# vpc-ccg/circminer

Hardware: AMD Instinct MI355X
Metric: paired reads/sec (whole node), hg38 k=20, 2x150 bp; circ_report bit-exact (higher is better)
Workload: dtype int32/u8 (chain scores f64)

## Files before the change

circminer_amd/csrc/cm_core.h:

```cpp
#pragma once
#include <stdint.h>

#include "circminer_hot.h"
#if defined(CM_STAGE2_HOST)
#include <vector>
#endif

#if defined(__HIPCC__)
#define CM_HD __host__ __device__
#define CM_NOINLINE inline
#else
#define CM_HD
#define CM_NOINLINE
#endif

#if !defined(CM_HOOK_DP)
#define CM_HOOK_DP(kind, s, n, t, m) ((void)0)
#endif
#if defined(CM_STATS) && !defined(__HIPCC__)
#if !defined(CM_NSTATS)
#define CM_NSTATS 16
#endif
extern "C" unsigned long long cm_stats[CM_NSTATS];
#define CM_STAT(i, n) ((i) < CM_NSTATS ? (void)(cm_stats[(i) < CM_NSTATS ? (i) : 0] += (unsigned long long)(n)) : (void)0)
// ... 59 lines not shown
};
struct AnnotV {
    uint32_t n_iv, n_seg, n_trans, n_gene, n_chr, iv_bucket_shift, n_iv_bucket, pair_reach;
    uint64_t n_bits;
    const CM_G IvRec *iv;
    g_u32 iv_seg;
    const CM_G SegRec *seg;
    g_u32 seg_tid;
    const CM_G TrRec *tr;
    g_u8 t2s;
    const CM_G GeneRec *gene;
    g_u64 near_border_bits, intronic_bits;
    g_u32 chr_shift;
    g_i32 chr_id;
    g_u32 iv_bucket;
};
CM_HD inline IndexV to_dev(const cm_index_view &v) {
    IndexV d;
    d.contig_num = v.contig_num; d.ref_len = v.ref_len; d.n_entries = v.n_entries;
    d.genome = (g_u8)v.genome; d.bucket_off = (g_u32)v.bucket_off; d.checksum = (g_u16)v.checksum; d.pos = (g_u32)v.pos;
    return d;
}
CM_HD inline AnnotV to_dev(const AnnotDev &v) {
    AnnotV d;
    d.n_iv = v.n_iv; d.n_seg = v.n_seg; d.n_trans = v.n_trans; d.n_gene = v.n_gene; d.n_chr = v.n_chr;
    d.iv_bucket_shift = v.iv_bucket_shift; d.n_iv_bucket = v.n_iv_bucket; d.n_bits = v.n_bits; d.pair_reach = v.pair_reach;
    d.iv = (const CM_G IvRec *)v.iv; d.iv_seg = (g_u32)v.iv_seg; d.seg = (const CM_G SegRec *)v.seg; d.seg_tid = (g_u32)v.seg_tid;
    d.tr = (const CM_G TrRec *)v.tr; d.t2s = (g_u8)v.t2s; d.gene = (const CM_G GeneRec *)v.gene;
    d.near_border_bits = (g_u64)v.near_border_bits; d.intronic_bits = (g_u64)v.intronic_bits;
    d.chr_shift = (g_u32)v.chr_shift; d.chr_id = (g_i32)v.chr_id; d.iv_bucket = (g_u32)v.iv_bucket;
    return d;
}

constexpr int INF_I = 1000000000;
constexpr uint32_t MINLB = 0u;
constexpr uint32_t MAXUB = 4294967295u;
constexpr int MAXDISCRDTLEN = 20000;
constexpr uint32_t LARIAT2BEGTH = 1000u;
constexpr int DPTINF = 10000000;
constexpr int SC_MAT = 1, SC_MIS = -3, SC_IND = -3, SC_XD = 8;
constexpr int MAX_SEEDS = CM_MAX_CHAIN_FRAGS;
constexpr int MAX_BAND = 8;
constexpr int MAX_TID = 64;
#if defined(CM_STAGE2_HOST)
constexpr int MEMO_N = 512;
#elif defined(CM_MEMO_N)
constexpr int MEMO_N = CM_MEMO_N;
#else
constexpr int MEMO_N = 8;
#endif

enum { ERR_POOL = 1, ERR_SEEDS = 4, ERR_BAND = 8, ERR_MEMO = 16 };

struct KCore {
    cm_params P;
    cm_index_view X;
    AnnotDev A;
    const uint32_t *desc = nullptr;
    const uint64_t *entry_near = nullptr;
};
struct Core {
    cm_params P;
    IndexV X;
    AnnotV A;
    g_u32 desc = nullptr;
    g_u64 entry_near = nullptr;
};
CM_HD inline Core to_core(const KCore &k) {
    Core c;
    c.P = k.P;
    c.X = to_dev(k.X);
    c.A = to_dev(k.A);
    c.desc = (g_u32)k.desc;
    c.entry_near = (g_u64)k.entry_near;
    return c;
}

template <class T> CM_HD inline T cmin(T a, T b) { return a < b ? a : b; }
template <class T> CM_HD inline T cmax(T a, T b) { return a > b ? a : b; }
CM_HD inline int cabs(int a) { return a < 0 ? -a : a; }

struct SV {
    g_u8 p;
    int32_t off;
    int32_t step;
    int32_t mode;
    CM_HD inline SV sub(int a) const { return SV{p, off + a * step, step, mode}; }
    CM_HD inline SV rev(int m) const { return SV{p, off + (m - 1) * step, -step, mode}; }
};
struct Read {
    g_u8 p;
    int32_t len;
    int32_t rc;
    CM_HD inline SV view() const { return rc ? SV{p, len - 1, -1, 1} : SV{p, 0, 1, 0}; }
};


struct Probe {
    uint32_t start;
    uint32_t raw;
    uint32_t touches;
};
template <class AT> CM_HD inline void probe_search(const AT &at, uint32_t n, int target, uint32_t b0, Probe &r) {
    uint32_t lb = 1, ub = n, mid;
    while (lb < ub) {
        mid = (lb + ub) / 2;
        ++r.touches;
        if (target <= at(mid - 1)) ub = mid;
        else lb = mid + 1;
    }
    ++r.touches;
    if (ub < lb || target != at(lb - 1)) return;
    const uint32_t LB = lb;
    uint32_t UB = lb;
    ub = n;
    while (lb < ub) {
        mid = (lb + ub + 1) / 2;
        ++r.touches;
        if (target < at(mid - 1)) ub = mid - 1;
        else lb = mid;
    }
    ++r.touches;
    if (target == at(lb - 1)) UB = lb;
    r.start = b0 + (LB - 1);
    r.raw = UB - LB + 1;
}
constexpr int DESC_WORDS = 4;
CM_HD inline int desc_cbits(int kmer) { return 2 * (kmer - CM_WINDOW_SIZE); }
CM_HD inline uint32_t desc_inline(int kmer) { return desc_cbits(kmer) > 0 ? (uint32_t)(88 / desc_cbits(kmer)) : 254u; }
CM_HD inline int desc_value(uint32_t d1, uint32_t d2, uint32_t d3, uint32_t i, int cbits) {
    const uint32_t sh = 8u + i * (uint32_t)cbits, w = sh >> 5, bit = sh & 31u;
    const uint32_t lo = w == 0 ? d1 : (w == 1 ? d2 : d3), hi = w == 0 ? d2 : (w == 1 ? d3 : 0u);
    const uint64_t two = ((uint64_t)hi << 32) | lo;
    return (int)((uint32_t)(two >> bit) & ((1u << cbits) - 1u));
}
template <class CK> CM_HD inline void desc_pack(uint32_t b0, uint32_t n, const CK &cks , int kmer, uint32_t out[DESC_WORDS]) {
    const int cbits = desc_cbits(kmer);
    uint64_t lo = n < 255u ? n : 255u;
    uint32_t hi = 0;
    if (n <= desc_inline(kmer) && cbits > 0)
        for (uint32_t i = 0; i < n; ++i) {
            const uint32_t sh = 8u + i * (uint32_t)cbits;
            const uint64_t v = (uint64_t)(cks(i) & ((1u << cbits) - 1u));
            if (sh < 64u) {
                lo |= v << sh;
                if (sh + (uint32_t)cbits > 64u) hi |= (uint32_t)(v >> (64u - sh));
            } else hi |= (uint32_t)(v << (sh - 64u));
        }
    out[0] = b0;
    out[1] = (uint32_t)lo;
    out[2] = (uint32_t)(lo >> 32);
    out[3] = hi;
}
CM_HD inline Probe seed_probe(const Core &c, const SV &s, int qpos) {
    Probe r{0u, 0u, 0u};
    int hv = 0, cv = 0;
    uint32_t bad = 0;
    const uint32_t rc = s.mode == 1 ? 1u : 0u;
    for (int i = 0; i < c.P.kmer; ++i) {
        uint32_t u = s.mode == 2 ? 0u : (uint32_t)s.p[s.off + (qpos + i) * s.step];
        u = rc ? (u & 0xDFu) : u;
        bad |= (uint32_t)!((u == 'A') | (u == 'C') | (u == 'G') | (u == 'T'));
        uint32_t code = ((u >> 1) ^ (u >> 2)) & 3u;
        code = rc ? 3u - code : code;
        if (i < CM_WINDOW_SIZE) hv = (hv << 2) | (int)code;
        else cv = (cv << 2) | (int)code;
    }
    if (bad) return r;
    const int target = (int)(int16_t)cv;
    if (c.desc) {
        const g_u32 d = c.desc + (uint64_t)(uint32_t)hv * DESC_WORDS;
        uint32_t w[DESC_WORDS];
        __builtin_memcpy(w, (const CM_G uint8_t *)d, sizeof(w));
        const uint32_t n8 = w[1] & 0xffu;
        if (n8 == 0) return r;
        if (n8 <= desc_inline(c.P.kmer)) {
            const int cbits = desc_cbits(c.P.kmer);
            const uint32_t d1 = w[1], d2 = w[2], d3 = w[3];
            probe_search([&](uint32_t i) { return cbits > 0 ? desc_value(d1, d2, d3, i, cbits) : 0; }, n8, target, w[0], r);
            return r;
        }
    }
    const uint32_t b0 = c.X.bucket_off[hv], b1 = c.X.bucket_off[hv + 1];
    if (b1 == b0) return r;
    const g_u16 it = c.X.checksum + b0;
    probe_search([&](uint32_t i) { return (int)it[i]; }, b1 - b0, target, b0, r);
    return r;
}

CM_HD inline bool bit_at(g_u64 b, uint64_t n, uint64_t p) { return p < n && ((b[p >> 6] >> (p & 63)) & 1ull); }
CM_HD inline uint32_t iv_nseg(const AnnotV &A, int iv) { return A.iv[iv].nseg; }
CM_HD inline uint32_t iv_segid(const AnnotV &A, int iv, uint32_t i) { return A.iv_seg[A.iv[iv].seg_off + i]; }

CM_HD inline int iv_find_ind(const AnnotV &A, uint32_t pos, int &ind) {
    CM_STAT(10, 1);
    ind = -1;
    if (pos < A.iv[0].spos) return -1;
    int beg = 0, end = (int)A.n_iv;
    const uint32_t b = pos >> A.iv_bucket_shift;
    if (A.iv_bucket && b + 1 < A.n_iv_bucket) {
        beg = (int)A.iv_bucket[b];
        end = (int)A.iv_bucket[b + 1];
        if (beg > 0) --beg;
        if (end < (int)A.n_iv) ++end;
        if (end <= beg) end = beg + 1;
    }
    while (end - beg > 1) {
        const int mid = (beg + end) / 2;
        if (pos < A.iv[mid].spos) end = mid;
        else beg = mid;
    }
    ind = end - 1;
    if (ind < 0 || A.iv[ind].epos < pos) return -1;
    return ind;
}
CM_HD inline int overlap_ind(const Core &c, uint32_t loc, int &ind) {
    int r = iv_find_ind(c.A, loc, ind);
    if (r < 0 || iv_nseg(c.A, r) == 0) return -1;
    return r;
}
CM_HD inline int overlap(const Core &c, uint32_t loc) { int ind; return overlap_ind(c, loc, ind); }

CM_HD inline uint32_t upper_bound_lookup(const Core &c, uint32_t spos, uint32_t mlen, uint32_t rlen, uint32_t &max_end, int &ol) {
    const AnnotV &A = c.A;
    max_end = 0;
    int it_ind = -1;
    int ov = iv_find_ind(A, spos, it_ind);
    const uint32_t epos = spos + mlen - 1;
    if (ov < 0 || iv_nseg(A, ov) == 0) {
        ol = -1;
        int nx = it_ind + 1;
        max_end = ((nx < 0 || nx >= (int)A.n_iv) ? 0u : A.iv[nx].spos) - 1u;
        if (max_end < epos) return 0;
        return cmin(spos + rlen + (uint32_t)c.P.max_ed, max_end - mlen + 1);
    }
    ol = -1;
    uint32_t min_end = 1000000000u, max_next = 0;
    if (epos > A.iv[ov].epos) {
        const uint32_t n = iv_nseg(A, ov);
        for (uint32_t i = 0; i < n; ++i) {
            uint32_t s = iv_segid(A, ov, i);
            uint32_t e = A.seg[s].end;
            if (e >= epos) {
                max_end = cmax(max_end, e);
                min_end = cmin(min_end, e);
                max_next = cmax(max_next, A.seg[s].next_exon_beg);
            }
        }
    } else {
        max_end = A.iv[ov].max_end;
        min_end = A.iv[ov].min_end;
        max_next = A.iv[ov].max_next_exon;
    }
    if (max_end > 0 && max_end >= epos) {
        ol = ov;
        if (min_end < rlen + epos && max_next != 0) return max_next + mlen - 1;
        return max_end - mlen + 1;
    }
    max_end = 0;
    ol = -1;
    return 0;
}
CM_HD inline uint32_t upper_bound(const Core &c, uint32_t spos, uint32_t mlen, uint32_t rlen, uint32_t &max_end, int &ol) {
    if (bit_at(c.A.near_border_bits, c.A.n_bits, spos)) return upper_bound_lookup(c, spos, mlen, rlen, max_end, ol);
    max_end = 0;
    ol = -1;
    return spos + rlen + (uint32_t)c.P.max_ed;
}
CM_HD inline int chr_row(const Core &c, uint32_t loc) {
    uint32_t i;
    for (i = 1; i < c.A.n_chr; ++i)
        if (loc < c.A.chr_shift[i]) return (int)i - 1;
    return (int)i - 1;
}

struct Event { double score; uint32_t cell; uint32_t pad; };
struct ChainWork {
    CM_G double *dp_score;
    CM_G int32_t *dp_prev;
    CM_G uint8_t *pool;
    unsigned long long pool_bytes;
    CM_G unsigned long long *pool_cursor;
    g_err err;
};

#if defined(__HIP_DEVICE_COMPILE__)
CM_HD inline unsigned long long pool_take(CM_G unsigned long long *cur, unsigned long long n) { return atomicAdd((unsigned long long *)cur, n); }
CM_HD inline void flag_err(g_err e, int bits) { atomicOr((int *)e, bits); }
#else
inline unsigned long long pool_take(unsigned long long *cur, unsigned long long n) { return __sync_fetch_and_add(cur, n); }
inline void flag_err(int *e, int bits) { __sync_fetch_and_or(e, bits); }
#endif

CM_HD inline bool check_junction(const Core &c, uint32_t s1, uint32_t s2, int ol, int kmer, int read_dist, int &trans_dist) {
    trans_dist = INF_I;
    if (ol < 0) return false;
    const uint32_t e1 = s1 + kmer - 1;
    if (s2 <= e1) return false;
    int td2intron = -1;
    const AnnotV &A = c.A;
    const uint32_t n = iv_nseg(A, ol);
    for (uint32_t i = 0; i < n; ++i) {
        const uint32_t s = iv_segid(A, ol, i);
        const int e12end = (int)(A.seg[s].end - e1);
        const int beg2s2 = (int)(s2 - A.seg[s].next_exon_beg);
        if (e12end >= 0 && e12end < read_dist && beg2s2 + kmer < 0) td2intron = (int)(s2 - e1 - 1);
        if (e12end < 0 || beg2s2 < 0) continue;
        trans_dist = e12end + beg2s2;
        if (cabs(trans_dist - read_dist) <= c.P.max_ed) return true;
    }
    if (td2intron != -1) {
        trans_dist = td2intron;
        return true;
    }
    trans_dist = INF_I;
    return false;
}

constexpr int SMALL_W = 32;
// ... 189 lines not shown
                int bl = (int)(cell >> 16);
                uint32_t bi = cell & 0xffffu;
                const uint32_t spos = S.pos(bl, bi);
                if (cur < best_score) {
                    bool rep = false;
                    for (uint32_t a = 0; a < best_count && !rep; ++a)
                        for (uint32_t b = 1; b < out[a].chain_len; ++b)
                            if (out[a].rpos[b] == spos) { rep = true; break; }
                    if (rep) continue;
                }
                CM_G cm_chain &ch = out[best_count++];
                uint32_t n = 0;
                while (true) {
                    ch.rpos[n] = S.pos(bl, bi);
                    ch.qpos[n] = bl * kmer;
                    ++n;
                    const int32_t pv = S.prev(S.base(bl) + bi);
                    if (pv < 0) break;
                    bl = (int)((uint32_t)pv >> 16);
                    bi = (uint32_t)pv & 0xffffu;
                }
                ch.score = (float)cur;
                ch.chain_len = n;
            }
            have = false;
            double nxt = 0;
            for (uint32_t q = 0; q < n_ev; ++q)
                if (S.ev_score(q) < cur && (!have || S.ev_score(q) > nxt)) {
                    nxt = S.ev_score(q);
                    have = true;
                }
            cur = nxt;
        }
    }
    if (best_count == 0) {
        for (int ii = kc - 1; ii >= 0; --ii)
            for (uint32_t i = 0; i < S.cnt(ii); ++i) {
                if (best_count >= max_best) break;
                CM_G cm_chain &ch = out[best_count++];
                ch.rpos[0] = S.pos(ii, i);
                ch.qpos[0] = ii * kmer;
                ch.score = (float)S.score(S.base(ii) + i);
                ch.chain_len = 1;
            }
    }
    return (int)best_count;
}

CM_HD inline int chain_kbest(const Core &c, int seq_len, int n_seeds, const uint32_t *start, const uint32_t *cnt, ChainWork &w, CM_G cm_chain *out) {
    int kc = n_seeds;
    while (kc >= 1 && cnt[kc - 1] == 0) --kc;
    if (kc <= 0) return 0;
    uint32_t base[MAX_SEEDS + 1];
    base[0] = 0;
    unsigned long long pairs = 0;
    for (int s = 0; s < kc; ++s) {
        pairs += (unsigned long long)cnt[s] * base[s];
        base[s + 1] = base[s] + cnt[s];
    }
    if (pairs <= (unsigned long long)SMALL_W && base[kc] <= (uint32_t)SMALL_W + 1u) {
        ChainStoreSmall S(c.X.pos, start, cnt, base, kc);
        return chain_kbest_t(c, seq_len, kc, S, out);
    }
    ChainStoreGlobal S(w, c.X.pos, start, cnt, base);
    return chain_kbest_t(c, seq_len, kc, S, out);
}

struct AlignRes { uint32_t pos; int ed, sclen, indel, qcovlen, rcovlen, score; };
struct MemoKey { uint32_t rspos, rlen, qspos, qlen; };
struct MemoSpill { MemoKey k; AlignRes v; };
typedef CM_G MemoSpill *g_spill;
CM_HD inline AlignRes ar_init(uint32_t p) { return AlignRes{p, 0, 0, 0, 0, 0, -INF_I}; }
CM_HD inline void ar_set(AlignRes &a, uint32_t p, int e, int s, int i, int qc, int scr) {
    a.pos = p; a.ed = e; a.sclen = s; a.indel = i; a.qcovlen = qc; a.rcovlen = qc - i; a.score = scr;
}
CM_HD inline void ar_update(AlignRes &a, int e, int s, uint32_t np, int i, int qc, int scr) {
    a.pos = np; a.ed += e; a.sclen = s; a.indel += i; a.qcovlen += qc; a.rcovlen += qc - i; a.score = scr;
}
CM_HD inline bool ar_by_score(AlignRes &b, const AlignRes &r, bool right) {
    const bool pos_better = right ? (r.pos < b.pos) : (r.pos > b.pos);
    if (b.score < r.score || (b.score == r.score && pos_better)) {
        ar_set(b, r.pos, r.ed, r.sclen, r.indel, r.qcovlen, r.score);
        return true;
    }
    return false;
}
CM_HD inline void ar_side(const Core &c, AlignRes &b, const AlignRes &r, bool right) {
    bool take = false;
    if (r.qcovlen > b.qcovlen) {
        take = r.ed <= c.P.max_ed && r.sclen <= c.P.max_sc && 2 * (r.ed - b.ed) < (r.qcovlen - b.qcovlen);
    } else if (r.qcovlen < b.qcovlen) {
        take = r.ed <= c.P.max_ed && r.sclen <= c.P.max_sc && 2 * (b.ed - r.ed) >= (b.qcovlen - r.qcovlen);
    } else {
        const bool pos_better = right ? (r.pos < b.pos) : (r.pos > b.pos);
        take = (r.ed < b.ed) || (r.ed == b.ed && r.sclen < b.sclen) || (r.ed == b.ed && r.sclen == b.sclen && pos_better);
    }
    if (take) ar_set(b, r.pos, r.ed, r.sclen, r.indel, r.qcovlen, r.score);
}
struct Cand { int ed, sclen, indel, score; };
CM_HD inline bool cand_less(const Cand &a, const Cand &b) {
    if (a.score != b.score) return a.score > b.score;
    if (a.ed != b.ed) return a.ed < b.ed;
    return cabs(a.indel) < cabs(b.indel);
}

#if defined(__HIP_DEVICE_COMPILE__)
constexpr int LSTRIDE = 64;
#else
constexpr int LSTRIDE = 1;
#endif
struct LBuf {
    CM_S uint8_t *b;
    int cap;
    CM_HD inline uint32_t word(int w) const {
#if defined(__HIP_DEVICE_COMPILE__)
        return ((CM_S const uint32_t *)b)[w * LSTRIDE];
#else
        uint32_t x;
        __builtin_memcpy(&x, b + 4 * w, 4);
        return x;
#endif
    }
    CM_HD inline uint8_t get(int i) const { return (uint8_t)((word(i >> 3) >> (4 * (i & 7))) & 0xFu); }
    CM_HD inline uint64_t window(int at) const {
        const int w = at >> 3;
        const uint64_t two = ((uint64_t)word(w + 1) << 32) | (uint64_t)word(w);
        uint64_t x = (uint32_t)(two >> (4 * (at & 7)));
        x = (x | (x << 16)) & 0x0000FFFF0000FFFFull;
        x = (x | (x << 8)) & 0x00FF00FF00FF00FFull;
        x = (x | (x << 4)) & 0x0F0F0F0F0F0F0F0Full;
        return x;
    }
    CM_HD inline void put(int i, uint8_t v) const {
        uint32_t x;
        __builtin_memcpy(&x, (const uint8_t *)b + 4 * (i >> 3) * LSTRIDE, 4);
        x = (x & ~(0xFu << (4 * (i & 7)))) | ((uint32_t)(v & 0xFu) << (4 * (i & 7)));
        __builtin_memcpy((uint8_t *)b + 4 * (i >> 3) * LSTRIDE, &x, 4);
    }
};
CM_HD inline uint32_t pack_nibbles(uint32_t x) { return (x & 0xFu) | ((x >> 4) & 0xF0u) | ((x >> 8) & 0xF00u) | ((x >> 12) & 0xF000u); }
CM_HD inline uint32_t swar_zero_bytes(uint32_t t) { return ~(((t & 0x7F7F7F7Fu) + 0x7F7F7F7Fu) | t | 0x7F7F7F7Fu); }
CM_HD inline uint32_t code4(uint32_t w, bool comp, uint8_t other) {
    const uint32_t x = w & 0xDFDFDFDFu;
    const uint32_t valid = swar_zero_bytes(x ^ 0x41414141u) | swar_zero_bytes(x ^ 0x43434343u) | swar_zero_bytes(x ^ 0x47474747u) |
                           swar_zero_bytes(x ^ 0x54545454u);
    const uint32_t m = (valid >> 7) * 0xFFu;
    uint32_t code = (x >> 1) & 0x03030303u;
    if (comp) code ^= 0x02020202u;
    return (code & m) | ((0x01010101u * other) & ~m);
}
CM_HD inline uint8_t code1(uint8_t ch, bool comp, uint8_t other) { return (uint8_t)(code4(ch, comp, other) & 0xFFu); }

constexpr int CM_STAGE_PAD = 64;
#if defined(__HIP_DEVICE_COMPILE__)
CM_HD inline void load_codes16(const SV &v, int w0, uint8_t other, uint32_t q[4]) {
    if (v.mode == 2) {
#pragma unroll
        for (int k = 0; k < 4; ++k) q[k] = 0x01010101u * other;
        return;
    }
    uint32_t r[4];
    if (v.step > 0) {
        __builtin_memcpy(r, (const CM_G uint8_t *)(v.p + v.off + 4 * w0), 16);
#pragma unroll
        for (int k = 0; k < 4; ++k) q[k] = code4(r[k], v.mode == 1, other);
    } else {
        __builtin_memcpy(r, (const CM_G uint8_t *)(v.p + v.off - 4 * w0 - 15), 16);
#pragma unroll
        for (int k = 0; k < 4; ++k) q[k] = code4(__builtin_bswap32(r[3 - k]), v.mode == 1, other);
    }
}
#endif
CM_HD inline void stage(const SV &v, int n, const LBuf &d, uint8_t other) {
    CM_STAT(8, 1);
#if defined(CM_ABL_NOSTAGE)
    return;
#endif
#if defined(__HIP_DEVICE_COMPILE__)
    CM_S uint32_t *dw = (CM_S uint32_t *)d.b;
    const int nw = (n + 7) >> 3;
    for (int w0 = 0; w0 < nw; w0 += 8) {
        uint32_t q[4][4];
#pragma unroll
        for (int u = 0; u < 4; ++u)
            if (w0 + 2 * u < nw) load_codes16(v, 2 * (w0 + 2 * u), other, q[u]);
#pragma unroll
        for (int u = 0; u < 4; ++u) {
            const int w = w0 + 2 * u;
            if (w < nw) dw[w * LSTRIDE] = pack_nibbles(q[u][0]) | (pack_nibbles(q[u][1]) << 16);
            if (w + 1 < nw) dw[(w + 1) * LSTRIDE] = pack_nibbles(q[u][2]) | (pack_nibbles(q[u][3]) << 16);
        }
    }
#else
    for (int i = 0; i < n; ++i) d.put(i, v.mode == 2 ? other : code1(v.p[v.off + i * v.step], v.mode == 1, other));
#endif
}
CM_HD inline int prefix_mismatches(const SV &a, const SV &b, int len) {
    int mm = 0;
#if defined(__HIP_DEVICE_COMPILE__)
    for (int w0 = 0; 4 * w0 < len; w0 += 4) {
        uint32_t qa[4], qb[4];
        load_codes16(a, w0, 4, qa);
        load_codes16(b, w0, 5, qb);
#pragma unroll
        for (int k = 0; k < 4; ++k) {
            const int base = 4 * (w0 + k);
            if (base >= len) continue;
            uint32_t x = qa[k] ^ qb[k];
            x = (x | (x >> 1) | (x >> 2)) & 0x01010101u;
            if (len - base < 4) x &= (1u << (8 * (len - base))) - 1u;
            mm += __builtin_popcount(x);
        }
    }
#else
    for (int i = 0; i < len; ++i) {
        const uint8_t x = a.mode == 2 ? 4 : code1(a.p[a.off + i * a.step], a.mode == 1, 4);
        const uint8_t y = b.mode == 2 ? 5 : code1(b.p[b.off + i * b.step], b.mode == 1, 5);
        mm += x != y;
    }
#endif
    return mm;
}
CM_HD inline bool prefix_equal(const SV &a, const SV &b, int len) {
#if defined(__HIP_DEVICE_COMPILE__)
    for (int w0 = 0; 4 * w0 < len; w0 += 4) {
        uint32_t qa[4], qb[4];
        load_codes16(a, w0, 4, qa);
        load_codes16(b, w0, 5, qb);
        uint32_t any = 0;
#pragma unroll
        for (int k = 0; k < 4; ++k) {
            const int base = 4 * (w0 + k);
            uint32_t x = qa[k] ^ qb[k];
            if (base >= len) x = 0;
            else if (len - base < 4) x &= (1u << (8 * (len - base))) - 1u;
            any |= x;
        }
        if (any) return false;
    }
    return true;
#else
    return prefix_mismatches(a, b, len) == 0;
#endif
}
CM_HD inline int ldiff(uint8_t a, uint8_t b) { return a == b ? 0 : 1; }
CM_HD inline int lscore(uint8_t a, uint8_t b) { return a == b ? SC_MAT : SC_MIS; }

constexpr int TINY = 4 * MAX_BAND + 4;
CM_HD inline void tiny_full_dp(const LBuf &s, int n, const LBuf &t, int m, int *col ) {
    for (int i = 0; i <= n; ++i) col[i] = i;
    for (int j = 1; j <= m; ++j) {
        int diag = col[0];
        col[0] = j;
        const uint8_t tj = t.get(j - 1);
        for (int i = 1; i <= n; ++i) {
            const int v = cmin(cmin(diag + ldiff(s.get(i - 1), tj), col[i - 1] + 1), col[i] + 1);
            diag = col[i];
            col[i] = v;
        }
    }
}

template <int WT> struct BandC { static constexpr int WC = WT > 0 ? WT : MAX_BAND; };

template <int WT>
CM_HD CM_NOINLINE int one_side_banded_impl(const LBuf &s, int n, const LBuf &t, int m, int w) {
    constexpr int WC = BandC<WT>::WC;
    if (w < 0 || n <= w) {
        int col[TINY];
        if (n >= TINY) n = TINY - 1;
        tiny_full_dp(s, n, t, m, col);
        return col[n];
    }
    int prev[WC + 3], cur[WC + 3];
#pragma unroll
    for (int x = 0; x < WC + 3; ++x) prev[x] = (x >= 1 && x <= w + 1) ? x - 1 : DPTINF;
    for (int i = 1; i <= n; ++i) {
        cur[0] = DPTINF;
        const uint8_t si = s.get(i - 1);
#pragma unroll
        for (int c = 0; c <= WC; ++c) {
            int v = DPTINF;
            if (c <= w) v = cmin(cmin(prev[c + 1] + ldiff(si, t.get(i + c - 1)), prev[c + 2] + 1), cur[c] + 1);
            cur[c + 1] = v;
        }
        cur[WC + 2] = DPTINF;
#pragma unroll
        for (int x = 0; x < WC + 3; ++x) prev[x] = cur[x];
    }
    int r = DPTINF;
#pragma unroll
    for (int x = 1; x <= WC + 1; ++x)
        if (x == (m - n) + 1) r = prev[x];
    return r;
}

template <int WT>
CM_HD CM_NOINLINE int local_alignment_side_impl(const Core &c, const LBuf &s, int n, const LBuf &t, int m, int &indel, int &align_score) {
    constexpr int WC = BandC<WT>::WC;
    const int w = WT > 0 ? WT : c.P.band;
    const int max_edit = c.P.max_ed;
    Cand best{max_edit + 1, c.P.max_sc + 1, w + 1, -1 * (c.P.max_sc + 1) - 2 * (max_edit + 1)};
    if (w < 0 || n <= 2 * w || m <= w) {
        int col[TINY];
        const int nn = n < TINY ? n : TINY - 1;
        tiny_full_dp(s, nn, t, m, col);
// ... 1528 lines not shown
```

circminer_amd/csrc/cm_hot.hip:

```cpp
#include <chrono>
#include <hip/hip_runtime.h>
#include <rocprim/device/device_radix_sort.hpp>

#include <algorithm>
#include <atomic>
#include <cstdarg>
#include <cstdio>
#include <cstdlib>
#include <cstring>
#include <string>
#include <functional>
#include <thread>
#include <vector>

#include "circminer_hot.h"
#include "cm_core.h"
#include "cm_aos.h"
#include "cm_index_build.h"
#include "cm_fastq_text.h"

using cmc::Core;
using cmc::KCore;

namespace {

constexpr int MAX_SLOTS = 16;
constexpr uint32_t TILE_PAIRS = 1u << 20;
constexpr uint32_t TILE_PAIRS_MAX = 1u << 21;
constexpr int BLK = 256;
constexpr int BLK_CHAIN = 64;
#include "cm_dp_engine.h"

enum ProfClass { PC_NONE = -1, PC_SEED = 0, PC_CHAIN = 1, PC_PAIR = 2, PC_SCAN = 3, PC_HEAVY = 4, PC_ORDER = 5, PC_CHAIN_HEAVY = 6, PC_PREFETCH = 7, PC_COUNT = 8 };
enum Counter {
    CN_PROBES = 0 , CN_PAIR_ROUNDS = 3, CN_RERUN = 4 ,
    CN_FALL = 5, CN_FALL_2ND = 6,
    CN_CD_LANE = 8, CN_CD_PHASE = 13, CN_CD_WAVE = 16, CN_CD_EVENTS = 20, CN_CD_LEVELS = 21, CN_CD_PROBLEMS = 22, CN_CD_PASSES = 23, CN_CD_CELLS = 24,
    CN_CD_REGLOG = 25, CN_CD_BATCHES = 26, CN_CD_PRE_USED = 27, CN_CD_PRE_UNUSED = 28,
    CN_HP_ATTEMPT = 8, CN_HP_STRIDE = 8, CN_HP_UNPAIRED = 24, CN_HP_CHAINS = 25, CN_HP_SEQ_TASKS = 26, CN_HP_EARLY = 27, CN_HP_EARLY_FIRST = 28,
    CN_WORDS = 32
};
static_assert(CN_CD_CELLS < CN_WORDS && CN_HP_EARLY_FIRST < CN_WORDS && CN_HP_ATTEMPT + CN_HP_STRIDE + 5 < CN_HP_UNPAIRED, "d_counters has CN_WORDS words");
enum Pin {
    PIN_COLLECT_N = 0, PIN_COLLECT_ERR = 1,
    PIN_DEV_ERR = 0,
    PIN_POOL_ERR = 2,
    PIN_HEAVY_LOAD = 4,
    PIN_CELLS = 8,
    PIN_RERUN_N = 12, PIN_FALL_N = 14,
    PIN_TEXT = 16,
    PIN_WORDS = 32
};
constexpr size_t PIN_BYTES = PIN_WORDS * sizeof(unsigned long long);
static_assert(PIN_BYTES == 256 && PIN_FALL_N + 1 < PIN_TEXT && PIN_CELLS + 3 < PIN_RERUN_N && PIN_TEXT + cmft::RES_WORDS <= PIN_WORDS, "the landing zone has 32 words");
struct ReadsDev {
    const uint8_t *seq1, *seq2;
    const uint64_t *off1, *off2;
};

__global__ void __launch_bounds__(BLK) k_seed(KCore kc, ReadsDev rd, const uint8_t *active, uint64_t pair0, uint32_t n_tile, int S,
                                              uint32_t *sstart, uint32_t *scnt, uint32_t *sraw, unsigned long long *counters) {
    const Core c = cmc::to_core(kc);
    __shared__ unsigned int sh[3];
    if (threadIdx.x < 3) sh[threadIdx.x] = 0;
    __syncthreads();
    const uint64_t q = (uint64_t)blockIdx.x * BLK + threadIdx.x;
    const uint64_t total = (uint64_t)n_tile * 4u * (uint64_t)S;
    if (q < total) {
        const uint32_t s = (uint32_t)(q % (uint64_t)S);
        const uint64_t r = q / (uint64_t)S;
        const int orient = (int)(r & 1u), mate = (int)((r >> 1) & 1u);
        const uint64_t p = pair0 + (r >> 2);
        uint32_t st = 0, cn = 0, rw = 0;
        if (active[p]) {
            const uint64_t o0 = mate ? rd.off2[p] : rd.off1[p], o1 = mate ? rd.off2[p + 1] : rd.off1[p + 1];
            const int len = (int)(o1 - o0);
            const int k = c.P.kmer;
            if ((int)(s + 1) * k <= len) {
                const cmc::Read R{(cmc::g_u8)((mate ? rd.seq2 : rd.seq1) + o0), len, orient};
                const cmc::Probe pr = cmc::seed_probe(c, R.view(), (int)s * k);
                st = pr.start;
                rw = pr.raw;
                cn = (pr.raw > (uint32_t)c.P.seed_lim) ? 0u : pr.raw;
                atomicAdd(&sh[0], 1u);
                atomicAdd(&sh[1], pr.touches);
                atomicAdd(&sh[2], cn);
            }
        }
        sstart[q] = st;
        scnt[q] = cn;
        sraw[q] = rw;
    }
    __syncthreads();
    if (threadIdx.x < 3 && sh[threadIdx.x]) atomicAdd(&counters[CN_PROBES + threadIdx.x], (unsigned long long)sh[threadIdx.x]);
}

constexpr int SCAN_T = 256;
constexpr int SCAN_ELEMS = 1024;
__global__ void __launch_bounds__(SCAN_T) k_scan_a(const uint32_t *scnt, int S, uint32_t n, unsigned long long *out, unsigned long long *bsum,
                                                   unsigned int *bmax) {
    __shared__ unsigned long long sh[SCAN_T];
    __shared__ unsigned int shmax;
    const uint32_t base = blockIdx.x * SCAN_ELEMS;
    unsigned long long run = 0;
    unsigned int my_max = 0;
    if (threadIdx.x == 0) shmax = 0;
#pragma unroll
    for (int k = 0; k < SCAN_ELEMS / SCAN_T; ++k) {
        const uint32_t r = base + k * SCAN_T + threadIdx.x;
        uint32_t c = 0;
        if (r < n)
            for (int s = 0; s < S; ++s) c += scnt[(uint64_t)r * S + s];
        my_max = c > my_max ? c : my_max;
        sh[threadIdx.x] = c;
        __syncthreads();
        for (int d = 1; d < SCAN_T; d <<= 1) {
            const unsigned long long x = (threadIdx.x >= (unsigned)d) ? sh[threadIdx.x - d] : 0ull;
            __syncthreads();
            sh[threadIdx.x] += x;
            __syncthreads();
        }
        if (r < n) out[r] = run + sh[threadIdx.x] - c;
        run += sh[SCAN_T - 1];
        __syncthreads();
    }
    atomicMax(&shmax, my_max);
    __syncthreads();
    if (threadIdx.x == 0) {
        bsum[blockIdx.x] = run;
        bmax[blockIdx.x] = shmax;
    }
}
template <class T, bool WITH_MAX>
__global__ void __launch_bounds__(1024) k_scan_mid(T *bsum, uint32_t nb, T *total, const unsigned int *bmax) {
    __shared__ T part[1024];
    __shared__ unsigned int gmax;
    const uint32_t t = threadIdx.x;
    const uint32_t chunk = (nb + 1023u) / 1024u;
    const uint32_t a = t * chunk, b = (a + chunk < nb) ? a + chunk : nb;
    T s = 0;
    unsigned int m = 0;
    if (WITH_MAX && t == 0) gmax = 0;
    if constexpr (WITH_MAX) __syncthreads();
    for (uint32_t i = a; i < b; ++i) {
        s += bsum[i];
        if constexpr (WITH_MAX) m = bmax[i] > m ? bmax[i] : m;
    }
    if constexpr (WITH_MAX) atomicMax(&gmax, m);
    part[t] = s;
    __syncthreads();
    for (uint32_t d = 1; d < 1024; d <<= 1) {
        const T v = (t >= d) ? part[t - d] : (T)0;
        __syncthreads();
        part[t] += v;
        __syncthreads();
    }
    T run = t ? part[t - 1] : (T)0;
    for (uint32_t i = a; i < b; ++i) {
        const T x = bsum[i];
        bsum[i] = run;
        run += x;
    }
    if (WITH_MAX && t == 1023) {
        total[0] = part[1023];
        total[1] = gmax;
    }
}
__global__ void __launch_bounds__(SCAN_T) k_scan_c(unsigned long long *out, const unsigned long long *bsum, uint32_t n) {
    const uint32_t i = blockIdx.x * SCAN_T + threadIdx.x;
    if (i < n) out[i] += bsum[i / SCAN_ELEMS];
}

__device__ inline int pack_resid(int left, int right) {
    left = left < 0 ? 0 : (left > 255 ? 255 : left);
    right = right < 0 ? 0 : (right > 255 ? 255 : right);
    return left | (right << 8);
}
#ifndef CM_CHAIN_WAVES
#define CM_CHAIN_WAVES 5
#endif
__global__ void __launch_bounds__(BLK_CHAIN, CM_CHAIN_WAVES) k_chain(KCore kc, ReadsDev rd, const uint8_t *active, uint64_t pair0, uint32_t r0, uint32_t r1, int S,
                                                     const uint32_t *sstart, const uint32_t *scnt, const uint32_t *sraw,
                                                     const unsigned long long *celloff, unsigned long long cellbase, double *dp_score,
                                                     int32_t *dp_prev, uint8_t *pool, unsigned long long pool_bytes,
                                                     unsigned long long *pool_cursor, cm_chain *chains, int32_t *nchain, int32_t *high, int *err,
                                                     uint16_t *resid, const uint32_t *perm, const unsigned int *perm_lo, const unsigned int *perm_hi) {
    uint32_t r = r0 + blockIdx.x * BLK_CHAIN + threadIdx.x;
    if (perm) {
        r += *perm_lo;
        if (r >= *perm_hi) return;
        r = perm[r];
    } else if (r >= r1) return;
    const Core c = cmc::to_core(kc);
    const uint64_t p = pair0 + (r >> 2);
    int n = 0, hh = 0, rs = 0;
    if (active[p]) {
        const int mate = (int)((r >> 1) & 1u);
        const uint64_t o0 = mate ? rd.off2[p] : rd.off1[p], o1 = mate ? rd.off2[p + 1] : rd.off1[p + 1];
        const int len = (int)(o1 - o0);
        uint32_t st[cmc::MAX_SEEDS], cn[cmc::MAX_SEEDS];
        for (int s = 0; s < S; ++s) {
            st[s] = sstart[(uint64_t)r * S + s];
            cn[s] = scnt[(uint64_t)r * S + s];
            if (sraw[(uint64_t)r * S + s] > 0 && cn[s] == 0) ++hh;
        }
        cmc::ChainWork w;
        w.dp_score = (CM_G double *)(dp_score + (celloff[r] - cellbase));
        w.dp_prev = (CM_G int32_t *)(dp_prev + (celloff[r] - cellbase));
        w.pool = (CM_G uint8_t *)pool;
        w.pool_bytes = pool_bytes;
        w.pool_cursor = (CM_G unsigned long long *)pool_cursor;
        w.err = (cmc::g_err)err;
        n = cmc::chain_kbest(c, len, S, st, cn, w, (CM_G cm_chain *)(chains + (uint64_t)r * CM_BESTCHAINLIM));
        if (n > 0) {
            const cm_chain &b = chains[(uint64_t)r * CM_BESTCHAINLIM];
            rs = pack_resid(b.qpos[0], len - (b.qpos[b.chain_len - 1] + c.P.kmer));
        }
    }
    nchain[r] = n;
    high[r] = hh;
    resid[r] = (uint16_t)rs;
}

struct RetryArgs {
    uint32_t *pair_err;
    uint32_t *list;
    unsigned int *count;
    cmc::MemoSpill *spill;
    int spill_cap;
    int first;
};

template <bool FIRST>
__device__ __forceinline__ void pair_kernel(const KCore &kc, const ReadsDev &rd, uint64_t pair0, uint32_t n_tile, const cm_chain *chains, const int32_t *nchain,
                                            const int32_t *high, cm_mapped_read *state, uint8_t *active, int32_t *cat, int is_last,
                                            int *err, unsigned long long *counters, int str_cap, unsigned long long *lane_clk,
                                            const uint32_t *perm, const unsigned int *n_light, unsigned int *next_chunk,
                                            const RetryArgs &ra) {
    const unsigned long long clk0 = lane_clk ? wall_clock64() : 0ull;
    extern __shared__ uint32_t lds_words[];
#if defined(CM_DIAG)
    __shared__ unsigned long long tick_w[65];
    cmc::Tick tick;
    for (int i = 0; i < 32; ++i) tick.acc[i] = 0;
// ... 3769 lines not shown
```

Measured before the change: 29.76 million.

## Vectorize k-mer encoding with 24-byte span loads and wave-reduce seed counters

seed_probe now loads a 24-byte span of the read as three 64-bit words and encodes the k-mer with SWAR bit tricks, including validity checking and reverse-complement handling. This replaces the per-character byte loop. In k_seed, the per-thread shared-memory atomics are replaced by DPP row reductions and readlane, so one lane per wavefront issues the atomics. The index math also uses 32-bit division when the total fits. Risks: the span reads past the end of the read (guarded by a padding static_assert), and the packed 16-bit touches counter could overflow within a wave.

```diff
diff --git a/circminer_amd/csrc/cm_core.h b/circminer_amd/csrc/cm_core.h
--- a/circminer_amd/csrc/cm_core.h
+++ b/circminer_amd/csrc/cm_core.h
@@ -235,19 +235,70 @@
     out[2] = (uint32_t)(lo >> 32);
     out[3] = hi;
 }
+constexpr int KMER_SPAN = 24;
+struct KmerCode { int hv, cv; uint32_t bad; };
+CM_HD inline KmerCode kmer_from_span(const uint64_t a[3], int k, uint32_t rc) {
+    uint64_t t[3];
+    if (rc) { t[0] = a[2]; t[1] = a[1]; t[2] = a[0]; }
+    else { t[0] = __builtin_bswap64(a[0]); t[1] = __builtin_bswap64(a[1]); t[2] = __builtin_bswap64(a[2]); }
+    const uint64_t ONES = 0x0101010101010101ull;
+    uint64_t all = 0, diff = 0;
+#pragma unroll
+    for (int j = 0; j < 3; ++j) {
+        const int nb = k - 8 * j;
+        const uint64_t keep = nb >= 8 ? ~0ull : (nb <= 0 ? 0ull : ~0ull << (8 * (8 - nb)));
+        const uint64_t u = rc ? (t[j] & 0xDFDFDFDFDFDFDFDFull) : t[j];
+        uint64_t code = ((u >> 1) ^ (u >> 2)) & (3u * ONES);
+        const uint64_t b0 = code & ONES, b1 = (code >> 1) & ONES, both = b0 & b1;
+        const uint64_t letter = (0x40u * ONES) | (both ^ ONES) | ((b0 ^ b1) << 1) | (b1 << 2) | (both << 4);
+        diff |= (u ^ letter) & keep;
+        code = (code | (code >> 6)) & 0x000F000F000F000Full;
+        code = (code | (code >> 12)) & 0x000000FF000000FFull;
+        code = (code | (code >> 24)) & 0xFFFFull;
+        all = (all << 16) | code;
+    }
+    if (rc) all ^= 0xFFFFFFFFFFFFull;
+    const uint64_t v = all >> (2 * (KMER_SPAN - k));
+    const int nc = k > CM_WINDOW_SIZE ? k - CM_WINDOW_SIZE : 0;
+    KmerCode r;
+    r.hv = (int)(uint32_t)(v >> (2 * nc));
+    r.cv = (int)(uint32_t)(v & ((1ull << (2 * nc)) - 1ull));
+    r.bad = diff != 0 ? 1u : 0u;
+    return r;
+}
+CM_HD inline g_u8 kmer_span_at(const SV &s, int qpos) { return s.mode == 1 ? s.p + s.off - qpos - (KMER_SPAN - 1) : s.p + s.off + qpos; }
 CM_HD inline Probe seed_probe(const Core &c, const SV &s, int qpos) {
     Probe r{0u, 0u, 0u};
     int hv = 0, cv = 0;
     uint32_t bad = 0;
     const uint32_t rc = s.mode == 1 ? 1u : 0u;
-    for (int i = 0; i < c.P.kmer; ++i) {
-        uint32_t u = s.mode == 2 ? 0u : (uint32_t)s.p[s.off + (qpos + i) * s.step];
-        u = rc ? (u & 0xDFu) : u;
-        bad |= (uint32_t)!((u == 'A') | (u == 'C') | (u == 'G') | (u == 'T'));
-        uint32_t code = ((u >> 1) ^ (u >> 2)) & 3u;
-        code = rc ? 3u - code : code;
-        if (i < CM_WINDOW_SIZE) hv = (hv << 2) | (int)code;
-        else cv = (cv << 2) | (int)code;
+    const int k = c.P.kmer;
+    if (k >= 1 && k <= KMER_SPAN && ((s.step == 1 && s.mode == 0) || (s.step == -1 && s.mode == 1))) {
+        uint64_t a[3];
+#if defined(__HIP_DEVICE_COMPILE__)
+        __builtin_memcpy(a, kmer_span_at(s, qpos), KMER_SPAN);
+#else
+        uint8_t span[KMER_SPAN] = {0};
+        for (int i = 0; i < k; ++i) span[rc ? KMER_SPAN - 1 - i : i] = s.p[s.off + (qpos + i) * s.step];
+        for (int j = 0; j < 3; ++j) {
+            a[j] = 0;
+            for (int b = 7; b >= 0; --b) a[j] = (a[j] << 8) | span[8 * j + b];
+        }
+#endif
+        const KmerCode kc = kmer_from_span(a, k, rc);
+        hv = kc.hv;
+        cv = kc.cv;
+        bad = kc.bad;
+    } else {
+        for (int i = 0; i < k; ++i) {
+            uint32_t u = s.mode == 2 ? 0u : (uint32_t)s.p[s.off + (qpos + i) * s.step];
+            u = rc ? (u & 0xDFu) : u;
+            bad |= (uint32_t)!((u == 'A') | (u == 'C') | (u == 'G') | (u == 'T'));
+            uint32_t code = ((u >> 1) ^ (u >> 2)) & 3u;
+            code = rc ? 3u - code : code;
+            if (i < CM_WINDOW_SIZE) hv = (hv << 2) | (int)code;
+            else cv = (cv << 2) | (int)code;
+        }
     }
     if (bad) return r;
     const int target = (int)(int16_t)cv;
@@ -743,6 +794,7 @@
 CM_HD inline uint8_t code1(uint8_t ch, bool comp, uint8_t other) { return (uint8_t)(code4(ch, comp, other) & 0xFFu); }
 
 constexpr int CM_STAGE_PAD = 64;
+static_assert(CM_STAGE_PAD >= KMER_SPAN, "seed_probe's word loads reach up to KMER_SPAN - 1 bytes outside a read");
 #if defined(__HIP_DEVICE_COMPILE__)
 CM_HD inline void load_codes16(const SV &v, int w0, uint8_t other, uint32_t q[4]) {
     if (v.mode == 2) {
diff --git a/circminer_amd/csrc/cm_hot.hip b/circminer_amd/csrc/cm_hot.hip
--- a/circminer_amd/csrc/cm_hot.hip
+++ b/circminer_amd/csrc/cm_hot.hip
@@ -66,30 +66,55 @@
     __syncthreads();
     const uint64_t q = (uint64_t)blockIdx.x * BLK + threadIdx.x;
     const uint64_t total = (uint64_t)n_tile * 4u * (uint64_t)S;
-    if (q < total) {
-        const uint32_t s = (uint32_t)(q % (uint64_t)S);
-        const uint64_t r = q / (uint64_t)S;
-        const int orient = (int)(r & 1u), mate = (int)((r >> 1) & 1u);
-        const uint64_t p = pair0 + (r >> 2);
-        uint32_t st = 0, cn = 0, rw = 0;
-        if (active[p]) {
-            const uint64_t o0 = mate ? rd.off2[p] : rd.off1[p], o1 = mate ? rd.off2[p + 1] : rd.off1[p + 1];
-            const int len = (int)(o1 - o0);
-            const int k = c.P.kmer;
-            if ((int)(s + 1) * k <= len) {
-                const cmc::Read R{(cmc::g_u8)((mate ? rd.seq2 : rd.seq1) + o0), len, orient};
-                const cmc::Probe pr = cmc::seed_probe(c, R.view(), (int)s * k);
-                st = pr.start;
-                rw = pr.raw;
-                cn = (pr.raw > (uint32_t)c.P.seed_lim) ? 0u : pr.raw;
-                atomicAdd(&sh[0], 1u);
-                atomicAdd(&sh[1], pr.touches);
-                atomicAdd(&sh[2], cn);
-            }
-        }
+    const bool in = q < total;
+    const uint64_t qc = in ? q : total - 1;
+    uint32_t s;
+    uint64_t r;
+    if ((total >> 32) == 0) {
+        s = (uint32_t)qc % (uint32_t)S;
+        r = (uint32_t)qc / (uint32_t)S;
+    } else {
+        s = (uint32_t)(qc % (uint64_t)S);
+        r = qc / (uint64_t)S;
+    }
+    const int orient = (int)(r & 1u), mate = (int)((r >> 1) & 1u);
+    const uint64_t p = pair0 + (r >> 2);
+    const uint8_t act = active[p];
+    uint64_t o[2];
+    __builtin_memcpy(o, (mate ? rd.off2 : rd.off1) + p, sizeof(o));
+    const int len = (int)(o[1] - o[0]);
+    const int k = c.P.kmer;
+    uint32_t st = 0, cn = 0, rw = 0, pt = 0;
+    if ((int)in & (int)(act != 0) & (int)((int)(s + 1) * k <= len)) {
+        const cmc::Read R{(cmc::g_u8)((mate ? rd.seq2 : rd.seq1) + o[0]), len, orient};
+        const cmc::Probe pr = cmc::seed_probe(c, R.view(), (int)s * k);
+        st = pr.start;
+        rw = pr.raw;
+        cn = (pr.raw > (uint32_t)c.P.seed_lim) ? 0u : pr.raw;
+        pt = 0x10000u | pr.touches;
+    }
+    if (in) {
         sstart[q] = st;
         scnt[q] = cn;
         sraw[q] = rw;
+    }
+    uint32_t a = pt, b = cn;
+#define CM_ROW_ADD(v, n) v += (uint32_t)__builtin_amdgcn_update_dpp(0, (int)v, 0x120 | (n), 0xF, 0xF, false)
+    CM_ROW_ADD(a, 1); CM_ROW_ADD(b, 1);
+    CM_ROW_ADD(a, 2); CM_ROW_ADD(b, 2);
+    CM_ROW_ADD(a, 4); CM_ROW_ADD(b, 4);
+    CM_ROW_ADD(a, 8); CM_ROW_ADD(b, 8);
+#undef CM_ROW_ADD
+    uint32_t wa = 0, wb = 0;
+#pragma unroll
+    for (int row = 0; row < 4; ++row) {
+        wa += (uint32_t)__builtin_amdgcn_readlane((int)a, 16 * row);
+        wb += (uint32_t)__builtin_amdgcn_readlane((int)b, 16 * row);
+    }
+    if ((threadIdx.x & 63u) == 0 && wa) {
+        atomicAdd(&sh[0], wa >> 16);
+        atomicAdd(&sh[1], wa & 0xFFFFu);
+        if (wb) atomicAdd(&sh[2], wb);
     }
     __syncthreads();
     if (threadIdx.x < 3 && sh[threadIdx.x]) atomicAdd(&counters[CN_PROBES + threadIdx.x], (unsigned long long)sh[threadIdx.x]);
```

Result: faster. 30.21 million, median of 6 (+1.5%).
